# CPJKU/beat_this

Hardware: NVIDIA H100
Metric: clips/sec (30 s audio->beats, final0) (higher is better)
Workload: dtype f16

## Files before the change

### beat_this_b200/csrc/kernels_attn.cu

```cuda
#include <cstdio>

#include "tc_common.cuh"

namespace bt {

constexpr int AT_BQ = 128;
constexpr int AT_BKV = 64;
constexpr int AT_NST = 4;
constexpr int AT_WARPS = 8;
constexpr int AT_THREADS = 32 * (AT_WARPS + 1);
constexpr int AT_SQ = AT_BQ * 64;
constexpr int AT_SKV = AT_BKV * 64;
constexpr int AT_SMEM = 1024 + AT_SQ + AT_NST * 2 * AT_SKV + 128;

constexpr uint32_t AT_POLY_MASK = 0x52u;

__device__ __forceinline__ uint32_t sw64_off(int r, int c) {
  return static_cast<uint32_t>(r * 64 + ((c ^ ((r >> 1) & 3)) << 4));
}

__global__ void __launch_bounds__(AT_THREADS, 2)
attn_time_kernel(const __grid_constant__ CUtensorMap tmQ, const __grid_constant__ CUtensorMap tmKV,
                 const float* __restrict__ gates, h16* __restrict__ out, int L, int heads,
                 const ChunkSrc* __restrict__ chunks, int seqs_per_chunk) {
  extern __shared__ uint8_t smem_raw[];
  const uint32_t sbase = (smem_u32(smem_raw) + 1023u) & ~1023u;
  const uint32_t sQ = sbase;
  const uint32_t sK = sQ + AT_SQ;
  const uint32_t sV = sK + AT_NST * AT_SKV;
  const uint32_t bar_q = sV + AT_NST * AT_SKV;
  const uint32_t full = bar_q + 8;
  const uint32_t empty = full + 8 * AT_NST;

  const int warp = threadIdx.x >> 5, lane = threadIdx.x & 31;
  const int q0 = blockIdx.x * AT_BQ;
  const int h = blockIdx.y;
  const int seq = blockIdx.z;
  const int C = heads * 32;
  const int Lk = chunks ? chunks[seq / seqs_per_chunk].len : L;
  const int nkv = ceil_div(Lk, AT_BKV);

  if (threadIdx.x == 0) {
    asm volatile("mbarrier.init.shared::cta.b64 [%0], %1;" ::"r"(bar_q), "r"(1));
    for (int i = 0; i < AT_NST; ++i) {
      asm volatile("mbarrier.init.shared::cta.b64 [%0], %1;" ::"r"(full + 8 * i), "r"(1));
      asm volatile("mbarrier.init.shared::cta.b64 [%0], %1;" ::"r"(empty + 8 * i), "r"(AT_WARPS));
    }
    fence_barrier_init();
  }
  __syncthreads();

  if (warp == AT_WARPS) {
    if (lane == 0) {
      tma_prefetch_desc(&tmQ);
      tma_prefetch_desc(&tmKV);
      mbar_expect_tx_a(bar_q, AT_SQ);
      tma_load_3d_a(sQ, &tmQ, bar_q, h * 32, q0, seq);
      for (int j = 0; j < nkv; ++j) {
        const int st = j % AT_NST;
        if (j >= AT_NST) mbar_wait_a(empty + 8 * st, ((j / AT_NST) - 1) & 1);
        mbar_expect_tx_a(full + 8 * st, 2 * AT_SKV);
        tma_load_3d_a(sK + st * AT_SKV, &tmKV, full + 8 * st, C + h * 32, j * AT_BKV, seq);
        tma_load_3d_a(sV + st * AT_SKV, &tmKV, full + 8 * st, 2 * C + h * 32, j * AT_BKV, seq);
      }
    }
    return;
  }

  const int r0 = warp * 16;
  mbar_wait_a(bar_q, 0);
  uint32_t qa[2][4];
#pragma unroll
  for (int ks = 0; ks < 2; ++ks) ldmatrix_x4(sQ + sw64_off(r0 + (lane & 15), 2 * ks + (lane >> 4)), qa[ks]);

  float o[4][4];
#pragma unroll
  for (int d = 0; d < 4; ++d) o[d][0] = o[d][1] = o[d][2] = o[d][3] = 0.f;
  float m_run[2] = {-INFINITY, -INFINITY}, l_run[2] = {0.f, 0.f};
  for (int j = 0; j < nkv; ++j) {
    const int st = j % AT_NST;
    mbar_wait_a(full + 8 * st, (j / AT_NST) & 1);
    const uint32_t kb = sK + st * AT_SKV, vb = sV + st * AT_SKV;
    float s[8][4];
#pragma unroll
    for (int nb = 0; nb < 8; ++nb) {
      s[nb][0] = s[nb][1] = s[nb][2] = s[nb][3] = 0.f;
      uint32_t kf[4];
      ldmatrix_x4(kb + sw64_off(nb * 8 + (lane & 7), lane >> 3), kf);
      mma_16816(s[nb], qa[0], kf[0], kf[1]);
      mma_16816(s[nb], qa[1], kf[2], kf[3]);
    }
    if (j == nkv - 1) {
      const int lim = Lk - j * AT_BKV;
#pragma unroll
      for (int nb = 0; nb < 8; ++nb) {
        const int key = nb * 8 + 2 * (lane & 3);
        if (key >= lim) s[nb][0] = s[nb][2] = -INFINITY;
        if (key + 1 >= lim) s[nb][1] = s[nb][3] = -INFINITY;
      }
    }
    float mx[2] = {-INFINITY, -INFINITY};
#pragma unroll
    for (int nb = 0; nb < 8; ++nb) {
      mx[0] = fmaxf(mx[0], fmaxf(s[nb][0], s[nb][1]));
      mx[1] = fmaxf(mx[1], fmaxf(s[nb][2], s[nb][3]));
    }
    float mref[2], alpha[2];
#pragma unroll
    for (int r = 0; r < 2; ++r) {
      mx[r] = fmaxf(mx[r], __shfl_xor_sync(0xffffffffu, mx[r], 1));
      mx[r] = fmaxf(mx[r], __shfl_xor_sync(0xffffffffu, mx[r], 2));
      mref[r] = fmaxf(m_run[r], mx[r]);
      alpha[r] = ex2_approx(m_run[r] - mref[r]);
      m_run[r] = mref[r];
      l_run[r] *= alpha[r];
    }
#pragma unroll
    for (int d = 0; d < 4; ++d) {
      o[d][0] *= alpha[0]; o[d][1] *= alpha[0];
      o[d][2] *= alpha[1]; o[d][3] *= alpha[1];
    }
    uint32_t pa[4][4];
#pragma unroll
    for (int nb = 0; nb < 8; ++nb) {
      float p[4];
#pragma unroll
      for (int i = 0; i < 4; ++i) {
        const float x = s[nb][i] - mref[i >> 1];
        p[i] = ((AT_POLY_MASK >> nb) & 1u) ? ex2_poly(x) : ex2_approx(x);
      }
      l_run[0] += p[0] + p[1];
      l_run[1] += p[2] + p[3];
      pa[nb >> 1][(nb & 1) * 2] = pack_h16x2(p[0], p[1]);
      pa[nb >> 1][(nb & 1) * 2 + 1] = pack_h16x2(p[2], p[3]);
    }
#pragma unroll
    for (int kk = 0; kk < 4; ++kk) {
      const int key = kk * 16 + (lane & 7) + ((lane >> 3) & 1) * 8;
#pragma unroll
      for (int dp = 0; dp < 2; ++dp) {
        uint32_t vf[4];
        ldmatrix_x4_trans(vb + sw64_off(key, 2 * dp + (lane >> 4)), vf);
        mma_16816(o[2 * dp], pa[kk], vf[0], vf[1]);
        mma_16816(o[2 * dp + 1], pa[kk], vf[2], vf[3]);
      }
    }
    __syncwarp();
    if (lane == 0) mbar_arrive_a(empty + 8 * st);
  }
#pragma unroll
  for (int r = 0; r < 2; ++r) {
    l_run[r] += __shfl_xor_sync(0xffffffffu, l_run[r], 1);
    l_run[r] += __shfl_xor_sync(0xffffffffu, l_run[r], 2);
  }
#pragma unroll
  for (int r = 0; r < 2; ++r) {
    const int q = q0 + r0 + (lane >> 2) + 8 * r;
    if (q < L) {
      const int64_t m = static_cast<int64_t>(seq) * L + q;
      const float gsc = gates[m * heads + h] / l_run[r];
      h16* dst = out + m * C + h * 32 + 2 * (lane & 3);
#pragma unroll
      for (int d = 0; d < 4; ++d)
        *reinterpret_cast<uint32_t*>(dst + 8 * d) = pack_h16x2(o[d][2 * r] * gsc, o[d][2 * r + 1] * gsc);
    }
  }
}

struct TcAttnPlan {
  CUtensorMap tmQ;
  CUtensorMap tmKV;
  int seqs, L, heads;
};

TcAttnPlan* tc_attn_plan_create(const void* qkv, int seqs, int L, int heads, char* err, int errlen) {
  TcAttnPlan* p = new TcAttnPlan();
  p->seqs = seqs; p->L = L; p->heads = heads;
  const int C = heads * 32;
  const uint64_t dims[3] = {static_cast<uint64_t>(3 * C), static_cast<uint64_t>(L), static_cast<uint64_t>(seqs)};
  const uint64_t strides[2] = {static_cast<uint64_t>(3 * C) * 2, static_cast<uint64_t>(L) * 3 * C * 2};
  const uint32_t box_q[3] = {32, AT_BQ, 1};
  const uint32_t box_kv[3] = {32, AT_BKV, 1};
  if (!make_tmap(&p->tmQ, qkv, 3, dims, strides, box_q, 64, err, errlen) ||
      !make_tmap(&p->tmKV, qkv, 3, dims, strides, box_kv, 64, err, errlen)) {
    delete p;
    return nullptr;
  }
  return p;
}
void tc_attn_plan_destroy(TcAttnPlan* p) { delete p; }

void launch_attn_time_tc(const TcAttnPlan* p, const float* gates, void* out, cudaStream_t st, const ChunkSrc* chunks,
                         int seqs_per_chunk) {
  dim3 grid(ceil_div(p->L, AT_BQ), p->heads, p->seqs);
  attn_time_kernel<<<grid, AT_THREADS, AT_SMEM, st>>>(p->tmQ, p->tmKV, gates, reinterpret_cast<h16*>(out), p->L, p->heads,
                                                      chunks, seqs_per_chunk);
}

int tc_init_attn(char* err, int errlen) {
  const cudaError_t r = cudaFuncSetAttribute(attn_time_kernel, cudaFuncAttributeMaxDynamicSharedMemorySize, AT_SMEM);
  if (r != cudaSuccess) {
    snprintf(err, errlen, "cudaFuncSetAttribute(attn_time_kernel) failed: %s", cudaGetErrorString(r));
    return -1;
  }
  return 0;
}

}
```

Baseline: 747.2.

## Fold TMA producer into consumer warp and precompute swizzled smem offsets

Removes the dedicated producer warp. Thread 0 now issues the first NST K/V loads up front, then refills one stage per iteration after waiting on the empty barrier, which lowers the thread count per block. Swizzled ldmatrix offsets are hoisted out of the loop as per-lane constants. The row-max reduction becomes a tree, and the output rescale is skipped when no row's max changed. The risk is that thread 0's blocking wait on the empty barrier stalls warp 0's compute, and the warp-uniform branch adds divergence checks.

```diff
diff --git a/beat_this_b200/csrc/kernels_attn.cu b/beat_this_b200/csrc/kernels_attn.cu
--- a/beat_this_b200/csrc/kernels_attn.cu
+++ b/beat_this_b200/csrc/kernels_attn.cu
@@ -8,7 +8,7 @@
 constexpr int AT_BKV = 64;
 constexpr int AT_NST = 4;
 constexpr int AT_WARPS = 8;
-constexpr int AT_THREADS = 32 * (AT_WARPS + 1);
+constexpr int AT_THREADS = 32 * AT_WARPS;
 constexpr int AT_SQ = AT_BQ * 64;
 constexpr int AT_SKV = AT_BKV * 64;
 constexpr int AT_SMEM = 1024 + AT_SQ + AT_NST * 2 * AT_SKV + 128;
@@ -39,54 +39,57 @@
   const int C = heads * 32;
   const int Lk = chunks ? chunks[seq / seqs_per_chunk].len : L;
   const int nkv = ceil_div(Lk, AT_BKV);
-
-  if (threadIdx.x == 0) {
+  const bool producer = threadIdx.x == 0;
+  auto load_kv = [&](int j) {
+    const int st = j % AT_NST;
+    mbar_expect_tx_a(full + 8 * st, 2 * AT_SKV);
+    tma_load_3d_a(sK + st * AT_SKV, &tmKV, full + 8 * st, C + h * 32, j * AT_BKV, seq);
+    tma_load_3d_a(sV + st * AT_SKV, &tmKV, full + 8 * st, 2 * C + h * 32, j * AT_BKV, seq);
+  };
+
+  if (producer) {
     asm volatile("mbarrier.init.shared::cta.b64 [%0], %1;" ::"r"(bar_q), "r"(1));
     for (int i = 0; i < AT_NST; ++i) {
       asm volatile("mbarrier.init.shared::cta.b64 [%0], %1;" ::"r"(full + 8 * i), "r"(1));
       asm volatile("mbarrier.init.shared::cta.b64 [%0], %1;" ::"r"(empty + 8 * i), "r"(AT_WARPS));
     }
     fence_barrier_init();
+    tma_prefetch_desc(&tmQ);
+    tma_prefetch_desc(&tmKV);
+    mbar_expect_tx_a(bar_q, AT_SQ);
+    tma_load_3d_a(sQ, &tmQ, bar_q, h * 32, q0, seq);
+    for (int j = 0; j < AT_NST && j < nkv; ++j) load_kv(j);
   }
   __syncthreads();
-
-  if (warp == AT_WARPS) {
-    if (lane == 0) {
-      tma_prefetch_desc(&tmQ);
-      tma_prefetch_desc(&tmKV);
-      mbar_expect_tx_a(bar_q, AT_SQ);
-      tma_load_3d_a(sQ, &tmQ, bar_q, h * 32, q0, seq);
-      for (int j = 0; j < nkv; ++j) {
-        const int st = j % AT_NST;
-        if (j >= AT_NST) mbar_wait_a(empty + 8 * st, ((j / AT_NST) - 1) & 1);
-        mbar_expect_tx_a(full + 8 * st, 2 * AT_SKV);
-        tma_load_3d_a(sK + st * AT_SKV, &tmKV, full + 8 * st, C + h * 32, j * AT_BKV, seq);
-        tma_load_3d_a(sV + st * AT_SKV, &tmKV, full + 8 * st, 2 * C + h * 32, j * AT_BKV, seq);
-      }
-    }
-    return;
-  }
 
   const int r0 = warp * 16;
   mbar_wait_a(bar_q, 0);
   uint32_t qa[2][4];
 #pragma unroll
   for (int ks = 0; ks < 2; ++ks) ldmatrix_x4(sQ + sw64_off(r0 + (lane & 15), 2 * ks + (lane >> 4)), qa[ks]);
+  uint32_t koff = sw64_off(lane & 7, lane >> 3);
+  const int vrow = (lane & 7) + ((lane >> 3) & 1) * 8;
+  uint32_t voff[2] = {sw64_off(vrow, lane >> 4), sw64_off(vrow, 2 + (lane >> 4))};
 
   float o[4][4];
 #pragma unroll
   for (int d = 0; d < 4; ++d) o[d][0] = o[d][1] = o[d][2] = o[d][3] = 0.f;
   float m_run[2] = {-INFINITY, -INFINITY}, l_run[2] = {0.f, 0.f};
   for (int j = 0; j < nkv; ++j) {
+    asm volatile("" : "+r"(koff), "+r"(voff[0]), "+r"(voff[1]));
+    if (producer && j > 0 && j + AT_NST - 1 < nkv) {
+      mbar_wait_a(empty + 8 * ((j - 1) % AT_NST), ((j - 1) / AT_NST) & 1);
+      load_kv(j + AT_NST - 1);
+    }
     const int st = j % AT_NST;
     mbar_wait_a(full + 8 * st, (j / AT_NST) & 1);
-    const uint32_t kb = sK + st * AT_SKV, vb = sV + st * AT_SKV;
+    const uint32_t kb = sK + st * AT_SKV + koff, vb = sV + st * AT_SKV;
     float s[8][4];
 #pragma unroll
     for (int nb = 0; nb < 8; ++nb) {
       s[nb][0] = s[nb][1] = s[nb][2] = s[nb][3] = 0.f;
       uint32_t kf[4];
-      ldmatrix_x4(kb + sw64_off(nb * 8 + (lane & 7), lane >> 3), kf);
+      ldmatrix_x4(kb + nb * 512, kf);
       mma_16816(s[nb], qa[0], kf[0], kf[1]);
       mma_16816(s[nb], qa[1], kf[2], kf[3]);
     }
@@ -99,26 +102,30 @@
         if (key + 1 >= lim) s[nb][1] = s[nb][3] = -INFINITY;
       }
     }
-    float mx[2] = {-INFINITY, -INFINITY};
+    float t[2][8];
 #pragma unroll
     for (int nb = 0; nb < 8; ++nb) {
-      mx[0] = fmaxf(mx[0], fmaxf(s[nb][0], s[nb][1]));
-      mx[1] = fmaxf(mx[1], fmaxf(s[nb][2], s[nb][3]));
+      t[0][nb] = fmaxf(s[nb][0], s[nb][1]);
+      t[1][nb] = fmaxf(s[nb][2], s[nb][3]);
     }
     float mref[2], alpha[2];
 #pragma unroll
     for (int r = 0; r < 2; ++r) {
-      mx[r] = fmaxf(mx[r], __shfl_xor_sync(0xffffffffu, mx[r], 1));
-      mx[r] = fmaxf(mx[r], __shfl_xor_sync(0xffffffffu, mx[r], 2));
-      mref[r] = fmaxf(m_run[r], mx[r]);
+#pragma unroll
+      for (int i = 0; i < 4; ++i) t[r][i] = fmaxf(t[r][i], t[r][i + 4]);
+      float mx = fmaxf(fmaxf(t[r][0], t[r][2]), fmaxf(t[r][1], t[r][3]));
+      mx = fmaxf(mx, __shfl_xor_sync(0xffffffffu, mx, 1));
+      mx = fmaxf(mx, __shfl_xor_sync(0xffffffffu, mx, 2));
+      mref[r] = fmaxf(m_run[r], mx);
       alpha[r] = ex2_approx(m_run[r] - mref[r]);
       m_run[r] = mref[r];
-      l_run[r] *= alpha[r];
-    }
-#pragma unroll
-    for (int d = 0; d < 4; ++d) {
-      o[d][0] *= alpha[0]; o[d][1] *= alpha[0];
-      o[d][2] *= alpha[1]; o[d][3] *= alpha[1];
+    }
+    if (__any_sync(0xffffffffu, alpha[0] != 1.f || alpha[1] != 1.f)) {
+#pragma unroll
+      for (int d = 0; d < 4; ++d) {
+        o[d][0] *= alpha[0]; o[d][1] *= alpha[0];
+        o[d][2] *= alpha[1]; o[d][3] *= alpha[1];
+      }
     }
     uint32_t pa[4][4];
 #pragma unroll
@@ -129,18 +136,17 @@
         const float x = s[nb][i] - mref[i >> 1];
         p[i] = ((AT_POLY_MASK >> nb) & 1u) ? ex2_poly(x) : ex2_approx(x);
       }
-      l_run[0] += p[0] + p[1];
-      l_run[1] += p[2] + p[3];
+      l_run[0] = nb == 0 ? fmaf(l_run[0], alpha[0], p[0] + p[1]) : l_run[0] + (p[0] + p[1]);
+      l_run[1] = nb == 0 ? fmaf(l_run[1], alpha[1], p[2] + p[3]) : l_run[1] + (p[2] + p[3]);
       pa[nb >> 1][(nb & 1) * 2] = pack_h16x2(p[0], p[1]);
       pa[nb >> 1][(nb & 1) * 2 + 1] = pack_h16x2(p[2], p[3]);
     }
 #pragma unroll
     for (int kk = 0; kk < 4; ++kk) {
-      const int key = kk * 16 + (lane & 7) + ((lane >> 3) & 1) * 8;
 #pragma unroll
       for (int dp = 0; dp < 2; ++dp) {
         uint32_t vf[4];
-        ldmatrix_x4_trans(vb + sw64_off(key, 2 * dp + (lane >> 4)), vf);
+        ldmatrix_x4_trans(vb + voff[dp] + kk * 1024, vf);
         mma_16816(o[2 * dp], pa[kk], vf[0], vf[1]);
         mma_16816(o[2 * dp + 1], pa[kk], vf[2], vf[3]);
       }
```

Result: faster. 775.9, median of 6 (+3.8%).
